# MystenLabs/dapol

Hardware: AMD Instinct MI355X
Metric: entities/sec (tree build + 64-bit range-proof gen), 2^20 leaves, 1/2/4/8 GPU (higher is better)
Workload: dtype int32 limbs (255-bit modular integers)

## Files before the change

dapol_amd/csrc/host_range.inc:

```

#include <cstdlib>
#include "policy_plan.inc"
#include "prove_plan.inc"

struct MsmTiming {
    std::vector<hipEvent_t> ev;
    std::vector<int> kind;
    size_t used = 0;
    bool enabled = false;
    size_t kernels[2] = {0, 0};
    ~MsmTiming() { for (auto e : ev) (void)hipEventDestroy(e); }
    hipError_t mark(hipStream_t st, int k = 0) {
        if (!enabled) return hipSuccess;
        if (used == ev.size()) {
            hipEvent_t e;
            hipError_t r = hipEventCreate(&e);
            if (r != hipSuccess) return r;
            ev.push_back(e);
        }
        if ((used & 1) == 0) { if (kind.size() <= used / 2) kind.push_back(k); else kind[used / 2] = k; }
        return hipEventRecord(ev[used++], st);
    }
    void count(int k, size_t n) { if (enabled) kernels[k] += n; }
    double total_ms(int k) {
// ... 38 lines not shown
static void launch_msm(hipStream_t st, const RangeArgs& A, const TableView& tv, int round, int lpl) {
    const unsigned B = (unsigned)A.B, S = (unsigned)(A.nsplit > 1 ? A.nsplit : 1);
    if (lpl == 8) hipLaunchKernelGGL((k_rp_msm<MSM_PLAIN, 8>), dim3((B + 3) / 4 * S), dim3(64), 0, st, A, tv, round);
    else if (lpl == 4) hipLaunchKernelGGL((k_rp_msm<MSM_PLAIN, 4>), dim3((B + 7) / 8 * S), dim3(64), 0, st, A, tv, round);
    else if (lpl == 2) hipLaunchKernelGGL((k_rp_msm<MSM_PLAIN, 2>), dim3((B + 15) / 16 * S), dim3(64), 0, st, A, tv, round);
    else if (lpl == 16) hipLaunchKernelGGL((k_rp_msm<MSM_PLAIN, 16>), dim3((B + 1) / 2 * S), dim3(64), 0, st, A, tv, round);
    else hipLaunchKernelGGL((k_rp_msm<MSM_PLAIN, 32>), dim3(B * S), dim3(64), 0, st, A, tv, round);
}
static void launch_msm_tail(hipStream_t st, const RangeArgs& At, const TableView& tvt, int round, int lpl) {
    const unsigned B = (unsigned)At.B;
    if (lpl == 2) hipLaunchKernelGGL((k_rp_msm<MSM_TAIL, 2>), dim3((B + 15) / 16), dim3(64), 0, st, At, tvt, round);
    else if (lpl == 1) hipLaunchKernelGGL((k_rp_msm<MSM_TAIL, 1>), dim3((B + 31) / 32), dim3(64), 0, st, At, tvt, round);
    else if (lpl == 32) hipLaunchKernelGGL((k_rp_msm<MSM_TAIL, 32>), dim3(B), dim3(64), 0, st, At, tvt, round);
    else if (lpl == 8) hipLaunchKernelGGL((k_rp_msm<MSM_TAIL, 8>), dim3((B + 3) / 4), dim3(64), 0, st, At, tvt, round);
    else hipLaunchKernelGGL((k_rp_msm<MSM_TAIL, 4>), dim3((B + 7) / 8), dim3(64), 0, st, At, tvt, round);
}

static size_t scratch_budget_bytes(const dapol_ctx* ctx = nullptr) {
    const double GiB = 1024.0 * 1024.0 * 1024.0;
    if (const char* e = knob("DAPOL_SCRATCH_GB")) {
        double gb = atof(e);
        if (gb < 0.25) gb = 0.25;
        return (size_t)(gb * GiB);
    }
    if (ctx && ctx->opt.scratch_gb > 0) return (size_t)((ctx->opt.scratch_gb < 0.25 ? 0.25 : ctx->opt.scratch_gb) * GiB);
    double want = (ctx && ctx->opt.profile == DAPOL_PROFILE_HOST ? 56.0 : 130.0) * GiB;
    size_t free_b = 0, total_b = 0;
    if (hipMemGetInfo(&free_b, &total_b) == hipSuccess) {
        double avail = (double)free_b + (ctx ? (double)ctx->scratch.bytes : 0.0) - 8.0 * GiB;
        if (avail < 0.25 * GiB) avail = 0.25 * GiB;
        if (avail < want) want = avail;
    }
    return (size_t)want;
}


static unsigned fold_blocks(const RangeArgs& A, size_t cb, int round) {
    if (!A.stab) return nblk(cb * (size_t)A.N, 256);
    const size_t half = (size_t)1 << (A.lgN - 1 - round), nt = (round + 1 <= STAB_ROUNDS) ? ((size_t)2 << (round + 1)) : 0;
    return nblk(cb * (half > nt ? half : nt), 256);
}

struct PendingProve {
    dapol_ctx* ctx = nullptr;
    DevBuf<uint32_t> err;
    int pinned_slot = 0;
    uint32_t* h_err_p = nullptr;
    bool armed = false;
    int32_t finish() {
        if (!armed) return DAPOL_OK;
        armed = false;
        HIPCHK(hipStreamSynchronize(ctx->stream));
        if (*h_err_p) return fail(DAPOL_ERR_INVALID_ARGUMENT, "prover drew a zero challenge (ProofError::MaliciousDealer)");
        return DAPOL_OK;
    }
    ~PendingProve() { if (armed) (void)hipStreamSynchronize(ctx->stream); }
};

struct ProveLane {
    RangeArgs A;
    int32_t* split[3];
    int32_t* gsacc;
};
static ProveLane carve_lane(const ProvePlan& P, RangeArgs A, uint8_t* base) {
    ProveLane L{};
    const size_t chunk = P.chunk, N = (size_t)P.N, T = (size_t)P.tail_n;
    size_t o = 0;
    A.a = (sc*)(base + o); o += chunk * N * sizeof(sc);
    A.b = (sc*)(base + o); o += chunk * N * sizeof(sc);
    A.s1 = (sc*)(base + o); o += chunk * N * sizeof(sc);
    A.s2 = (sc*)(base + o); o += chunk * N * sizeof(sc);
    A.dig = (dig_t*)(base + o); o += align_up(chunk * P.dig_elems * sizeof(dig_t), 256);
    A.st = (ProofState*)(base + o); o += align_up(chunk * sizeof(ProofState), 256);
    A.PA = (int32_t*)(base + o); o += chunk * 160;
    A.P0 = (int32_t*)(base + o); o += chunk * 160;
    A.P1 = (int32_t*)(base + o); o += chunk * 160;
    A.tailT = (int32_t*)(base + o); o += chunk * 2 * T * TAIL_ROW_WORDS * 4;
    A.tail_a = (sc*)(base + o); o += chunk * T * sizeof(sc);
    A.tail_b = (sc*)(base + o); o += chunk * T * sizeof(sc);
    A.tail_s1 = (sc*)(base + o); o += chunk * T * sizeof(sc);
    A.tail_s2 = (sc*)(base + o); o += chunk * T * sizeof(sc);
    A.fs_part = (sc*)(base + o); o += chunk * FS_PARTS_MAX * 3 * sizeof(sc);
    A.stab = P.stab_bytes ? (sc*)(base + o) : nullptr; o += chunk * P.stab_bytes;
    L.gsacc = (int32_t*)(base + o); o += chunk * P.acc_bytes;
    o = align_up(o, 256);
    L.split[0] = (int32_t*)(base + o); o += chunk * (size_t)P.part_split() * 160;
    L.split[1] = (int32_t*)(base + o); o += chunk * (size_t)P.part_split() * 160;
    o = align_up(o, 256);
    L.split[2] = (int32_t*)(base + o);
    L.A = A;
    return L;
}

static void launch_main_msm(dapol_ctx* ctx, const ProvePlan& P, const ProveLane& L, const RangeArgs& A, hipStream_t st, int round, MsmTiming* tm) {
    const size_t cb = A.B;
    if (P.gs) {
        const int LW = P.gs_LW;
        const unsigned g_acc = nblk(cb * (size_t)LW, 64);
        const int ns = P.slices_for(cb), slice_rows = A.N / ns, tile = P.tile_for(cb, ns);
        const size_t side_words = (size_t)4 * FE_NL * cb * LW * ns;
        for (int side = 0; side < 2; side++)
            for (int q0 = 0; q0 < slice_rows; q0 += tile) {
                const int nq = slice_rows - q0 < tile ? slice_rows - q0 : tile;
                if (LW < A.nwin)
                    hipLaunchKernelGGL(k_rp_msm_gs_hi, dim3(g_acc, ns), dim3(64), 0, st, A, ctx->tv, round, side, q0, nq, q0 == 0 ? 1 : 0,
                                       L.gsacc + side * side_words, slice_rows, LW);
                else
                    hipLaunchKernelGGL(k_rp_msm_gs, dim3(g_acc, ns), dim3(64), 0, st, A, ctx->tv, round, side, q0, nq, q0 == 0 ? 1 : 0,
                                       L.gsacc + side * side_words, slice_rows);
            }
        if (ns > 1) hipLaunchKernelGGL(k_rp_gs_sum_slices, dim3(nblk(2 * cb * (size_t)LW, 64)), dim3(64), 0, st, A, L.gsacc, side_words, ns, LW);
        hipLaunchKernelGGL(k_rp_gs_combine, dim3(nblk(2 * cb, 64)), dim3(64), 0, st, A, L.gsacc, side_words, ns, LW);
        if (tm) tm->count(0, 2 * (size_t)((slice_rows + tile - 1) / tile));
    } else if (P.part_split() > 1) {
        RangeArgs As = A;
        As.nsplit = P.part_split(); As.P0 = L.split[0]; As.P1 = L.split[1];
        if (P.quad_split) hipLaunchKernelGGL(k_rp_msm_quad, dim3((unsigned)(cb * (size_t)P.quad_split)), dim3(64), 0, st, As, ctx->tv, round);
        else launch_msm(st, As, ctx->tv, round, P.lpl);
        hipLaunchKernelGGL(k_rp_sum_splits, dim3((unsigned)(2 * cb)), dim3(64), 0, st, cb, As.nsplit, As.P0, As.P1, A.P0, A.P1);
    } else {
        launch_msm(st, A, ctx->tv, round, P.lpl);
        if (tm) tm->count(0, 1);
    }
}

static int32_t launch_materialise(dapol_ctx* ctx, const ProvePlan& P, const ProveLane& L, const RangeArgs& A, hipStream_t st, MsmTiming* tm) {
    const size_t cb = A.B, T = (size_t)P.tail_n;
    const unsigned g_tail = (unsigned)(cb * (size_t)(P.tail_n / 32));
    if (P.gs_mat) {
        const int LW = P.mat_LW(), cpl = P.mat_cpl(cb);
        const unsigned g_cls = nblk(cb * (size_t)LW, 64);
        const size_t slot_words = (size_t)4 * FE_NL * cb * LW;
        for (int side = 0; side < 2; side++)
            for (int c0 = 0; c0 < P.tail_n; c0 += MAT_GROUP) {
                const int nc = P.tail_n - c0 < MAT_GROUP ? P.tail_n - c0 : MAT_GROUP;
                for (int c = 0; c < nc; c += cpl) {
                    const int ny = nc - c < cpl ? nc - c : cpl;
                    hipLaunchKernelGGL(k_rp_mat_gs, dim3(g_cls, ny), dim3(64), 0, st, A, ctx->tv, side, c0 + c, 0, LW, L.gsacc + c * slot_words);
                    if (LW < A.nwin) hipLaunchKernelGGL(k_rp_mat_gs, dim3(g_cls, ny), dim3(64), 0, st, A, ctx->tv, side, c0 + c, 1, LW, L.gsacc + c * slot_words);
                }
                hipLaunchKernelGGL(k_rp_mat_gs_horner, dim3(nblk(cb * (size_t)nc, 64)), dim3(64), 0, st, A, side, c0, nc, LW, L.gsacc);
            }
        if (tm) tm->count(1, 2 * (size_t)((P.tail_n + cpl - 1) / cpl) * (LW < A.nwin ? 2 : 1));
    } else if (P.mat_split > 1) {
        RangeArgs Am = A;
        Am.nsplit = P.mat_split; Am.P0 = L.split[2];
        hipLaunchKernelGGL((k_rp_msm<MSM_MATERIALIZE, 32>), dim3(g_tail * (unsigned)P.mat_split), dim3(64), 0, st, Am, ctx->tv, -1); LAUNCH_CHECK();
        hipLaunchKernelGGL(k_rp_sum_mat, dim3(nblk(cb * 2 * T, 64)), dim3(64), 0, st, cb * 2 * T, P.mat_split, Am.P0, A.tailT);
    } else {
        hipLaunchKernelGGL((k_rp_msm<MSM_MATERIALIZE, 32>), dim3(g_tail), dim3(64), 0, st, A, ctx->tv, -1);
        if (tm) tm->count(1, 1);
    }
    LAUNCH_CHECK();
    return DAPOL_OK;
}

static int32_t queue_chunk(dapol_ctx* ctx, const ProvePlan& P, const ProveLane& L, RangeArgs A, hipStream_t st, ForkGuard& fg, uint32_t* d_err,
                           MsmTiming* tm) {
    const size_t cb = A.B;
    const int fs_shape = P.fs_shape, nf_rounds = P.nf_rounds();
    sc* const stab_buf = A.stab;
    if (!P.stab_main) A.stab = nullptr;
    const unsigned g_wave = (unsigned)cb, g_lane = nblk(cb, 64), g_dig = (unsigned)(cb * (size_t)(A.TP / 64));
    const unsigned g_gsdig = nblk(cb * (size_t)(2 * A.N), 64);
    hipLaunchKernelGGL(k_rp_nonce_key, dim3(g_lane), dim3(64), 0, st, A); LAUNCH_CHECK();
    if (P.gs) hipLaunchKernelGGL(k_rp_nonces_gs, dim3(g_gsdig), dim3(64), 0, st, A);
    else hipLaunchKernelGGL(k_rp_nonces, dim3(g_dig), dim3(64), 0, st, A);
    LAUNCH_CHECK();
    if (P.side_A) {
        HIPCHK(hipEventRecord(ctx->ev_fork, st));
        HIPCHK(hipStreamWaitEvent(ctx->side[2], ctx->ev_fork, 0));
        fg.forked(2);
        hipLaunchKernelGGL(k_rp_A, dim3(g_wave), dim3(64), 0, ctx->side[2], A, ctx->tv); LAUNCH_CHECK();
        HIPCHK(hipEventRecord(ctx->ev_join[2], ctx->side[2]));
        FAULT_AFTER_FORK("prove_A");
    } else if (P.a_lane(cb)) {
        hipLaunchKernelGGL(k_rp_A_lane, dim3(g_lane), dim3(64), 0, st, A, ctx->tv); LAUNCH_CHECK();
    } else {
        hipLaunchKernelGGL(k_rp_A, dim3(g_wave), dim3(64), 0, st, A, ctx->tv); LAUNCH_CHECK();
    }
    if (tm) HIPCHK(tm->mark(st));
    launch_main_msm(ctx, P, L, A, st, -1, tm); LAUNCH_CHECK();
    if (tm) HIPCHK(tm->mark(st));
    if (P.side_A) { HIPCHK(hipStreamWaitEvent(st, ctx->ev_join[2], 0)); fg.joined(2); }
    LAUNCH_FS(k_rp_finish1, fs_shape, cb, st, A, ctx->tv); LAUNCH_CHECK();
    hipLaunchKernelGGL(k_rp_poly, dim3(g_wave * (unsigned)A.fs_parts), dim3(64), 0, st, A); LAUNCH_CHECK();
    LAUNCH_FS(k_rp_finish2, fs_shape, cb, st, A, ctx->tv); LAUNCH_CHECK();
    hipLaunchKernelGGL(k_rp_lr, dim3(g_wave * (unsigned)A.fs_parts), dim3(64), 0, st, A); LAUNCH_CHECK();
    if (fs_shape == 2) hipLaunchKernelGGL(k_rp_finish3<2>, dim3(g_wave), dim3(64), 0, st, A);
    else hipLaunchKernelGGL(k_rp_finish3<0>, dim3(g_lane), dim3(64), 0, st, A);
    LAUNCH_CHECK();
    for (int k = 0; k < nf_rounds; k++) {
        if (P.gs) hipLaunchKernelGGL(k_rp_round_prep_gs, dim3(g_gsdig), dim3(64), 0, st, A, k);
        else hipLaunchKernelGGL(k_rp_round_prep, dim3(g_dig), dim3(64), 0, st, A, k);
        LAUNCH_CHECK();
        hipLaunchKernelGGL(k_rp_round_ip, dim3(g_wave), dim3(64), 0, st, A, k); LAUNCH_CHECK();
        if (tm) HIPCHK(tm->mark(st));
        launch_main_msm(ctx, P, L, A, st, k, tm); LAUNCH_CHECK();
        if (tm) HIPCHK(tm->mark(st));
        LAUNCH_FS(k_rp_round_finish, fs_shape, cb, st, A, ctx->tv, k); LAUNCH_CHECK();
        hipLaunchKernelGGL(k_rp_fold, dim3(fold_blocks(A, cb, k)), dim3(256), 0, st, A, k);
        LAUNCH_CHECK();
    }
    if (nf_rounds == A.lgN) {
        hipLaunchKernelGGL(k_rp_final, dim3(g_lane), dim3(64), 0, st, A, d_err); LAUNCH_CHECK();
        return DAPOL_OK;
    }
    if (P.gs_mat) hipLaunchKernelGGL(k_rp_mat_prep_gs, dim3(g_gsdig), dim3(64), 0, st, A);
    else hipLaunchKernelGGL(k_rp_mat_prep, dim3(g_dig), dim3(64), 0, st, A);
    LAUNCH_CHECK();
    if (tm) HIPCHK(tm->mark(st, 1));
    { int32_t rc = launch_materialise(ctx, P, L, A, st, tm); if (rc) return rc; }
    if (tm) HIPCHK(tm->mark(st, 1));
    const unsigned g_tail = (unsigned)(cb * (size_t)(P.tail_n / 32));
    {
        RangeArgs Ai = A;
        Ai.stab = P.stab_tail ? stab_buf : nullptr;
        hipLaunchKernelGGL(k_rp_tail_table, dim3(g_tail), dim3(64), 0, st, Ai); LAUNCH_CHECK();
    }
    RangeArgs At = A;
    At.N = P.tail_n; At.lgN = P.tail_lgn; At.TP = 2 * P.tail_n; At.wbits = TAIL_WBITS; At.nwin = TAIL_NWIN; At.nsplit = 0;
    At.a = A.tail_a; At.b = A.tail_b; At.s1 = A.tail_s1; At.s2 = A.tail_s2;
    At.stab = P.stab_tail ? stab_buf : nullptr;
    At.out_round0 = nf_rounds;
    const TableView tvt{A.tailT, 1, TAIL_WBITS, 0, 0};
    for (int k = 0; k < P.tail_lgn; k++) {
        hipLaunchKernelGGL(k_rp_round_prep, dim3(g_tail), dim3(64), 0, st, At, k); LAUNCH_CHECK();
        hipLaunchKernelGGL(k_rp_round_ip, dim3(g_wave), dim3(64), 0, st, At, k); LAUNCH_CHECK();
        launch_msm_tail(st, At, tvt, k, P.tail_lpl); LAUNCH_CHECK();
        LAUNCH_FS(k_rp_round_finish, fs_shape, cb, st, At, ctx->tv, k); LAUNCH_CHECK();
        hipLaunchKernelGGL(k_rp_fold, dim3(fold_blocks(At, cb, k)), dim3(256), 0, st, At, k);
        LAUNCH_CHECK();
    }
    hipLaunchKernelGGL(k_rp_final, dim3(g_lane), dim3(64), 0, st, At, d_err); LAUNCH_CHECK();
    return DAPOL_OK;
}

static int32_t range_prove_device(dapol_ctx* ctx, int n, int m, size_t B, const uint64_t* d_vals, const uint32_t* d_blind,
                                  const uint32_t* d_Vc, const uint32_t* d_seed, const uint64_t* d_stream, uint64_t slot_base,
                                  const uint32_t* d_tape, uint32_t* d_out, MsmTiming* tm, size_t tape_stride = 0, uint32_t sub_k = 1,
                                  size_t out_stride = 0, PendingProve* pend = nullptr) {
    ProveShape s{};
    s.n = n; s.m = m; s.B = B;
    s.tail_length = ctx->opt.tail_length; s.small_call_max = ctx->opt.small_call_max; s.generator_stationary = ctx->opt.generator_stationary;
    s.streams = ctx->opt.streams; s.gs_tile_rows = ctx->opt.gs_tile_rows; s.gs_slices = ctx->opt.gs_slices; s.chunk_proofs = ctx->opt.chunk_proofs;
    s.wbits = ctx->tv.wbits; s.nwin = ctx->tv.nwin_c(); s.hi_split = ctx->tv.hi_split;
    s.n_cu = ctx->n_cu; s.resident_waves = ctx->resident_waves();
    s.budget_bytes = scratch_budget_bytes(ctx);
    s.timed = tm != nullptr;
    ProvePlan P = plan_range_prove(s);
    for (bool lowered = false;; lowered = true) {
        hipError_t e = ctx->scratch.ensure(P.lane_bytes() * P.nlanes);
        if (e == hipSuccess) {
            if (lowered) P.finalise(s, P.chunk, P.nlanes);
            break;
        }
        (void)hipGetLastError();
        if (e != hipErrorOutOfMemory || (P.nlanes == 1 && P.chunk <= 64)) return fail_hip(e, "scratch allocation", __FILE__, __LINE__);
        if (P.nlanes > 1) P.nlanes--;
        else P.chunk = (P.chunk + 1) / 2;
    }
    const size_t chunk = P.chunk, slots = (size_t)m * (2 * (size_t)n + 4);
    const int nlanes = P.nlanes;
    RangeArgs A{};
    A.n = n; A.m = m; A.N = P.N; A.lgN = P.lgN; A.TP = P.TP;
    A.out_words = 72 + 16 * A.lgN;
    A.seed = d_seed; A.slot_base = slot_base;
    A.wbits = s.wbits; A.nwin = s.nwin;
    A.tail_n = P.tail_n; A.use_hi = P.use_hi ? 1 : 0; A.fs_parts = P.fs_parts; A.mat_round = P.nf_rounds();
    A.stream_id = d_stream;
    A.tape_stride = (uint32_t)(tape_stride ? tape_stride : slots);
    A.tape = d_tape;
    A.sub_k = sub_k ? sub_k : 1; A.sub_slots = (uint32_t)slots;
    A.out = d_out; A.out_stride = out_stride ? out_stride : (size_t)A.out_words;
    ProveLane lanes[4];
    hipStream_t lane_stream[4] = {ctx->stream, ctx->side[0], ctx->side[1], ctx->side[2]};
    for (int ln = 0; ln < nlanes; ln++) lanes[ln] = carve_lane(P, A, (uint8_t*)ctx->scratch.p + P.lane_bytes() * ln);
    DevBuf<uint32_t> err_own;
    DevBuf<uint32_t>& err = pend ? pend->err : err_own;
    HIPCHK(err.alloc(1));
    HIPCHK(hipMemsetAsync(err.p, 0, 4, ctx->stream));
    ForkGuard fg(ctx);
    if (nlanes > 1) {
        HIPCHK(hipEventRecord(ctx->ev_fork, ctx->stream));
        for (int ln = 1; ln < nlanes; ln++) { HIPCHK(hipStreamWaitEvent(lane_stream[ln], ctx->ev_fork, 0)); fg.forked(ln - 1); }
    }
    size_t chunk_no = 0;
    for (size_t first = 0; first < B; first += chunk, chunk_no++) {
        const int ln = (int)(chunk_no % (size_t)nlanes);
        if (chunk_no == 2) FAULT_AFTER_FORK("prove_lanes");
        RangeArgs Ac = lanes[ln].A;
        Ac.B = B - first < chunk ? B - first : chunk;
        Ac.vals = d_vals + first * m;
        Ac.blind = d_blind + first * m * 8;
        Ac.Vc = d_Vc + first * m * 8;
        Ac.p0 = first;
        int32_t rc = queue_chunk(ctx, P, lanes[ln], Ac, lane_stream[ln], fg, err.p, tm);
        if (rc) return rc;
    }
    for (int ln = 1; ln < nlanes; ln++) {
        HIPCHK(hipEventRecord(ctx->ev_join[ln - 1], lane_stream[ln]));
        HIPCHK(hipStreamWaitEvent(ctx->stream, ctx->ev_join[ln - 1], 0));
        fg.joined(ln - 1);
    }
    if (pend) {
        pend->ctx = ctx;
        pend->h_err_p = ctx->h_pinned + pend->pinned_slot;
        HIPCHK(hipMemcpyAsync(pend->h_err_p, err.p, 4, hipMemcpyDeviceToHost, ctx->stream));
        pend->armed = true;
        return DAPOL_OK;
    }
    uint32_t h_err = 0;
// ... 52 lines not shown
```

dapol_amd/csrc/kernels_range.h:

```cpp
#pragma once
#include <hip/hip_runtime.h>
#include <type_traits>
#include "kernels_ctx_tree.h"
#include "ge_quad.h"

namespace dapol {

struct ProofState {
    uint64_t strobe[25];
    uint32_t pos, pos_begin;
    uint32_t err, pad_;
    sc y, z, y_inv, x, w, u, u_inv;
    sc a_bl, s_bl, t1, t2, t1_bl, t2_bl, t_x, cL, cR;
    uint32_t nkey[8];
};

struct RangeArgs {
    int n, m, N, lgN, TP;
    int wbits, nwin;
    size_t B;
    const uint64_t* vals;
    const uint32_t* blind;
    const uint32_t* Vc;
    const uint32_t* seed;
// ... 380 lines not shown
            fe qel;
            for (int i = 0; i < FE_NL; i++) qel.v[i] = e[i];
            quad_madd(c, ql, qel, neg);
        }
    }
    for (int off = 16; off >= 4; off >>= 1) {
        fe o;
        for (int i = 0; i < FE_NL; i++) o.v[i] = __shfl_down(c.v[i], off, 64);
        quad_add(c, ql, o);
    }
    if (sub == 0) {
        int32_t* dst = (side ? A.P1 : A.P0) + (b * nsplit + split) * 40 + FE_NL * ql;
        for (int i = 0; i < FE_NL; i++) dst[i] = c.v[i];
    }
}

__global__ __launch_bounds__(64) void k_rp_sum_splits(size_t B, int nsplit, const int32_t* PS0, const int32_t* PS1, int32_t* P0, int32_t* P1) {
    const size_t t = blockIdx.x;
    if (t >= 2 * B) return;
    const size_t b = t >> 1;
    const int l = threadIdx.x;
    const int32_t* src = ((t & 1) ? PS1 : PS0) + b * (size_t)nsplit * 40;
    ge_p3 acc;
    if (l < nsplit) ld_p3(acc, src + (size_t)l * 40);
    else ge_identity(acc);
    for (int s = l + 64; s < nsplit; s += 64) {
        ge_p3 p, r;
        ld_p3(p, src + (size_t)s * 40);
        ge_add(r, acc, p);
        acc = r;
    }
    wave_reduce_point(acc, nsplit < 64 ? nsplit : 64);
    if (l == 0) st_p3(((t & 1) ? P1 : P0) + b * 40, acc);
}

__global__ __launch_bounds__(64) void k_rp_sum_mat(size_t n_gen, int nsplit, const int32_t* PS, int32_t* tailT) {
    size_t g = (size_t)blockIdx.x * 64 + threadIdx.x;
    if (g >= n_gen) return;
    const int32_t* src = PS + g * (size_t)nsplit * 40;
    ge_p3 acc, p, r;
    ld_p3(acc, src);
    for (int s = 1; s < nsplit; s++) {
        ld_p3(p, src + (size_t)s * 40);
        ge_add(r, acc, p);
        acc = r;
    }
    st_p3(tailT + g * TAIL_ROW_WORDS, acc);
}

template <int ENTRIES>
__device__ __forceinline__ void build_niels_row(int32_t* row) {
    ge_p3 base, mul;
    ld_p3(base, row);
    mul = base;
    fe pre[ENTRIES - 1];
#pragma unroll
    for (int e = 1; e < ENTRIES; e++) {
        if (e > 1) { ge_p3 t; ge_add(t, mul, base); mul = t; }
        int32_t* slot = row + e * 32;
        for (int i = 0; i < FE_NL; i++) { slot[i] = mul.X.v[i]; slot[FE_NL + i] = mul.Y.v[i]; slot[2 * FE_NL + i] = mul.Z.v[i]; }
        if (e == 1) pre[0] = mul.Z;
        else fe_mul(pre[e - 1], pre[e - 2], mul.Z);
    }
    fe inv;
    fe_invert(inv, pre[ENTRIES - 2]);
#pragma unroll
    for (int e = ENTRIES - 1; e >= 1; e--) {
        int32_t* slot = row + e * 32;
        fe X, Y, Z, zi, x, y;
        for (int i = 0; i < FE_NL; i++) { X.v[i] = slot[i]; Y.v[i] = slot[FE_NL + i]; Z.v[i] = slot[2 * FE_NL + i]; }
        if (e > 1) { fe_mul(zi, inv, pre[e - 2]); fe t; fe_mul(t, inv, Z); inv = t; }
        else zi = inv;
        fe_mul(x, X, zi);
        fe_mul(y, Y, zi);
        ge_niels q;
        ge_to_niels(q, x, y);
        niels_store_entry(slot, q);
    }
    ge_niels id;
    ge_niels_identity(id);
    niels_store_entry(row, id);
}

__global__ __launch_bounds__(64) void k_rp_tail_table(RangeArgs A) {
    const int T = A.tail_n, bpp = (2 * T) >> 6;
    size_t b = blockIdx.x / bpp;
    int g = (int)(blockIdx.x % bpp) * 64 + threadIdx.x;
    build_niels_row<TAIL_ENTRIES>(A.tailT + (b * (size_t)(2 * T) + g) * TAIL_ROW_WORDS);
    sc one, v;
    sc_zero(one); one.v[0] = 1;
    int i = g < T ? g : g - T;
    if (g == 0) stab_init(A, b);
    st_sc((g < T ? A.tail_s1 : A.tail_s2) + b * T + i, one);
    ld_sc(v, (g < T ? A.a : A.b) + b * A.N + i);
    st_sc((g < T ? A.tail_a : A.tail_b) + b * T + i, v);
}

__global__ __launch_bounds__(64) void k_rp_mat_prep(RangeArgs A) {
    int nch = A.TP >> 6;
    size_t b = blockIdx.x / nch;
    int ch = blockIdx.x % nch, l = threadIdx.x, side = l >> 5, q = 32 * ch + (l & 31), pos = 64 * ch + l;
    if (q >= A.N) { zero_digits(A, b, pos); return; }
    sc s;
    coeff_plain(s, A, b, A.mat_round, q, side != 0);
    write_digits_plain(A, b, pos, s.v);
}

__device__ __forceinline__ void st_load(Strobe& s, const ProofState& p) {
    for (int i = 0; i < 25; i++) s.s[i] = p.strobe[i];
    s.pos = p.pos;
    s.pos_begin = p.pos_begin;
}
__device__ __forceinline__ void st_store(ProofState& p, const Strobe& s) {
    for (int i = 0; i < 25; i++) p.strobe[i] = s.s[i];
    p.pos = s.pos;
    p.pos_begin = s.pos_begin;
}
__device__ __forceinline__ void st_load(WStrobe& s, const ProofState& p) {
    s.a = s.l < 25 ? p.strobe[s.l < 25 ? s.l : 0] : 0;
    s.pos = p.pos;
    s.pos_begin = p.pos_begin;
}
__device__ __forceinline__ void st_store(ProofState& p, const WStrobe& s) {
    if (s.l < 25) p.strobe[s.l] = s.a;
    if (s.l == 0) { p.pos = s.pos; p.pos_begin = s.pos_begin; }
}
template <class S>
__device__ __forceinline__ void challenge_scalar(sc& r, S& s, const char* label, int n) {
    uint32_t w[16];
    merlin_challenge_wide(s, label, n, w);
    sc_from_wide(r, w);
}
template <class S>
__device__ __forceinline__ void append_scalar(S& s, const char* label, int n, const uint32_t* canon8) {
    merlin_append_words(s, label, n, canon8, 8);
}
__device__ __forceinline__ void fs_scalar(sc& r, const RangeArgs& A, size_t b, int which) {
    const ProofState& ps = A.st[b];
    if (A.fs_parts > 1) {
        sc_zero(r);
        for (int w = 0; w < A.fs_parts; w++) {
            sc t;
            ld_sc(t, A.fs_part + (b * A.fs_parts + w) * 3 + which);
            sc_add(r, r, t);
        }
    } else {
        r = which == 0 ? ps.t1 : which == 1 ? ps.t2 : ps.t_x;
    }
}
template <int MODE> struct FsShape {
    using strobe_t = typename std::conditional<MODE == 2, WStrobe, Strobe>::type;
    const int l;
    size_t b;
    bool valid;
    int h_lo, h_hi;
    __device__ FsShape(const RangeArgs& A) : l((int)threadIdx.x) {
        const size_t t_ = (size_t)blockIdx.x * 64 + threadIdx.x;
        b = MODE == 2 ? (size_t)blockIdx.x : (MODE == 1 ? t_ >> 1 : t_);
        valid = b < A.B;
        if (!valid) b = A.B - 1;
        if (MODE == 0) { h_lo = 0; h_hi = 2; }
        else if (MODE == 1) { h_lo = (int)(t_ & 1); h_hi = h_lo + 1; }
        else { h_lo = l >> 5; h_hi = h_lo + 1; }
    }
    __device__ void share(uint32_t* first8, uint32_t* second8) const {
        if (MODE == 1) { for (int i = 0; i < 8; i++) second8[i] = (uint32_t)__shfl_down((int)second8[i], 1, 64); }
        if (MODE == 2) {
            for (int i = 0; i < 8; i++) { first8[i] = (uint32_t)__shfl((int)first8[i], 0, 64); second8[i] = (uint32_t)__shfl((int)second8[i], 32, 64); }
        }
    }
    __device__ bool point_lane() const { return MODE == 2 ? (l & 31) == 0 : true; }
    __device__ bool owns_transcript() const { return MODE == 2 ? true : (MODE == 1 ? ((l & 1) == 0 && valid) : valid); }
    __device__ bool writes() const { return MODE == 2 ? l == 0 : true; }
    __device__ void begin(strobe_t& s) const { if constexpr (MODE == 2) wstrobe_lanes(s, l); }
};
template <int MODE>
__device__ __forceinline__ void blinding_sum(sc& bl, const RangeArgs& A, size_t b, uint32_t slot0, uint32_t stride, int lane) {
    sc t;
// ... 472 lines not shown
```

dapol_amd/csrc/kernels_range_gs.h:

```cpp
#pragma once
#include "kernels_range.h"

namespace dapol {

__device__ __forceinline__ void write_digits_gs(const RangeArgs& A, size_t p, int sp, const uint32_t* c) {
    const size_t L = A.B * (size_t)A.nwin;
    int32_t* out = reinterpret_cast<int32_t*>(A.dig) + ((((size_t)(sp >> 2)) * L + p) << 2) + (sp & 3);
    const size_t wstride = A.B * (size_t)4;
    const int W = A.wbits, NW = A.nwin, half = 1 << (W - 1);
    const uint32_t mask = (1u << W) - 1;
    uint32_t x[8];
#pragma unroll
    for (int i = 0; i < 8; i++) x[i] = c[i];
    int carry = 0;
#pragma nounroll
    for (int w = 0; w < NW; w++) {
        const int b = (int)(x[0] & mask) + carry;
        carry = (b >= half && w != NW - 1) ? 1 : 0;
        out[(size_t)w * wstride] = b - (carry << W);
#pragma unroll
        for (int i = 0; i < 7; i++) x[i] = (x[i] >> W) | (x[i + 1] << (32 - W));
        x[7] >>= W;
    }
}
// ... 183 lines not shown
enum { GS_ACC_SLOTS = 32, GS_MAX_SLICES = 16, GS_FULL_LANES = 3072 * 64 };
static_assert(GS_ACC_SLOTS >= MAT_GROUP && GS_ACC_SLOTS >= 2 * GS_MAX_SLICES, "accumulator slots");

__global__ __launch_bounds__(64) void k_rp_mat_prep_gs(RangeArgs A) {
    GS_BLOCKS(A, vb) {
        size_t p;
        int sp;
        if (!gs_thread(A, vb, p, sp)) continue;
        const int side = sp >= A.N ? 1 : 0, rem = sp - side * A.N;
        const int per = A.N / A.tail_n, cls = rem / per, k = rem - cls * per;
        sc s;
        coeff_plain(s, A, p, A.mat_round, cls + k * A.tail_n, side != 0);
        write_digits_gs(A, p, sp, s.v);
    }
}

__global__ __launch_bounds__(64, DAPOL_GS_OCC) void k_rp_mat_gs(RangeArgs A, TableView tbl, int side, int cls, int hi, int LW, int32_t* __restrict__ accs) {
    const size_t LM = A.B * (size_t)LW, L = A.B * (size_t)A.nwin;
    const size_t lane = (size_t)blockIdx.x * 64 + threadIdx.x;
    if (lane >= LM) return;
    cls += (int)blockIdx.y;
    accs += (size_t)blockIdx.y * 4 * FE_NL * LM;
    const int w = (int)(lane / A.B);
    const size_t p = lane - (size_t)w * A.B;
    const int wd = w + (hi ? LW : 0);
    if (wd >= A.nwin) return;
    ge_p3 acc;
    int32_t* ap = accs + lane;
    if (!hi) ge_identity(acc);
    else {
#pragma unroll
        for (int i = 0; i < FE_NL; i++) {
            acc.X.v[i] = ap[(size_t)i * LM]; acc.Y.v[i] = ap[(size_t)(FE_NL + i) * LM];
            acc.Z.v[i] = ap[(size_t)(2 * FE_NL + i) * LM]; acc.T.v[i] = ap[(size_t)(3 * FE_NL + i) * LM];
        }
    }
    const int per = A.N / A.tail_n;
    const dapol_v4i* dg = reinterpret_cast<const dapol_v4i*>(A.dig) + ((size_t)(side * A.N + cls * per) >> 2) * L + (size_t)wd * A.B + p;
    dapol_v4i d4 = dg[0], dn = d4;
#pragma nounroll
    for (int k = 0; k < per; k++) {
        if ((k & 3) == 0 && k + 4 < per) dn = dg[(size_t)((k >> 2) + 1) * L];
        const int d = d4.x;
        d4.x = d4.y; d4.y = d4.z; d4.z = d4.w;
        if ((k & 3) == 3) d4 = dn;
        const int row = gen_row(tbl, A.n, cls + k * A.tail_n, side != 0);
        tbl_madd(acc, tbl, hi ? tbl.row_hi(row) : row, d);
    }
#pragma unroll
    for (int i = 0; i < FE_NL; i++) {
        ap[(size_t)i * LM] = acc.X.v[i]; ap[(size_t)(FE_NL + i) * LM] = acc.Y.v[i];
        ap[(size_t)(2 * FE_NL + i) * LM] = acc.Z.v[i]; ap[(size_t)(3 * FE_NL + i) * LM] = acc.T.v[i];
    }
}

__global__ __launch_bounds__(64) void k_rp_mat_gs_horner(RangeArgs A, int side, int cls0, int ncls, int LW, const int32_t* __restrict__ accs) {
    const size_t LM = A.B * (size_t)LW;
    const size_t t = (size_t)blockIdx.x * 64 + threadIdx.x;
    if (t >= (size_t)ncls * A.B) return;
    const int c = (int)(t / A.B);
    const size_t p = t - (size_t)c * A.B;
    const int32_t* slot = accs + (size_t)c * 4 * FE_NL * LM;
    auto load = [&](ge_p3& r, int w) {
        const int32_t* ap = slot + (size_t)w * A.B + p;
        for (int i = 0; i < FE_NL; i++) {
            r.X.v[i] = ap[(size_t)i * LM]; r.Y.v[i] = ap[(size_t)(FE_NL + i) * LM];
            r.Z.v[i] = ap[(size_t)(2 * FE_NL + i) * LM]; r.T.v[i] = ap[(size_t)(3 * FE_NL + i) * LM];
        }
    };
    ge_p3 acc, q, r;
    load(acc, LW - 1);
#pragma nounroll
    for (int w = LW - 2; w >= 0; w--) {
#pragma nounroll
        for (int d = 0; d < A.wbits; d++) ge_dbl(acc, acc, d == A.wbits - 1);
        load(q, w);
        ge_add(r, acc, q);
        acc = r;
    }
    const int T = A.tail_n;
    st_p3(A.tailT + (p * (size_t)(2 * T) + (size_t)(side * T + cls0 + c)) * TAIL_ROW_WORDS, acc);
}

}
```

dapol_amd/csrc/prove_plan.inc:

```
#pragma once
#include <cstddef>
#include <cstdint>
#include <cstdlib>

enum { FS_PARTS_MAX = 8 };

struct ProveShape {
    int n, m;
    size_t B;
    int tail_length, small_call_max, generator_stationary, streams, gs_tile_rows, gs_slices;
    long long chunk_proofs;
    int wbits, nwin, hi_split;
    int n_cu;
    size_t resident_waves;
    size_t budget_bytes;
    bool timed;
};

struct ProvePlan {
    int N, lgN, TP;
    int nwin, hi_split;
    int tail_n, tail_lgn;
    bool small_call, use_hi;
    int fs_shape, fs_parts;
    bool gs, gs_mat;
    int gs_LW, acc_slots;
    bool stab_main, stab_tail;
    int msm_split, mat_split, quad_split;
    size_t dig_elems, stab_bytes, acc_bytes, per_proof, split_bytes;
    size_t chunk;
    int nlanes;
    bool big_batch;
    int lpl, tail_lpl;
    bool side_A;
    int gs_tile, gs_slices_forced, mat_cpl_forced;
    bool gs_tile_set, a_lane_ok;
    const char* lpl_env;

    int part_split() const { return quad_split ? quad_split : msm_split; }
    int nf_rounds() const { return lgN - tail_lgn; }
    size_t lane_bytes() const { return (chunk * per_proof + 8192 + split_bytes + 4095) / 4096 * 4096; }

    int slices_for(size_t cb) const {
        if (gs_slices_forced) return gs_slices_forced <= acc_slots / 2 ? gs_slices_forced : acc_slots / 2;
        int ns = cb <= 4096 ? 16 : (cb < 40000 ? 8 : (cb < 65536 ? 4 : 1));
        if (N < 1024) {
            const size_t lanes = cb * (size_t)gs_LW;
            ns = lanes >= 2 * (size_t)GS_FULL_LANES ? 1 : (lanes >= (size_t)GS_FULL_LANES ? 2 : (lanes >= (size_t)GS_FULL_LANES / 2 ? 4 : (lanes >= (size_t)GS_FULL_LANES / 8 ? 8 : 16)));
        }
        while (ns > 1 && ((N / ns) % 4 != 0 || N / ns < 32)) ns /= 2;
        return ns;
    }
    int tile_for(size_t cb, int ns) const {
        int tile = (!gs_tile_set && cb * (size_t)nwin < 2 * (size_t)GS_FULL_LANES && N / ns >= 32) ? 32 : gs_tile;
        if (gs_LW < nwin && !gs_tile_set) tile = tile / 2;
        return tile;
    }
    int mat_LW() const { return hi_split ? hi_split : nwin; }
    int mat_cpl(size_t cb) const {
        if (mat_cpl_forced) return mat_cpl_forced;
        int cpl = 1;
        while (cpl < MAT_GROUP && cb * (size_t)mat_LW() * (size_t)cpl < GS_FULL_LANES) cpl *= 2;
        return cpl;
    }
    bool a_lane(size_t cb) const { return !side_A && gs && N < 1024 && cb >= 4096 && a_lane_ok; }

    void finalise(const ProveShape& s, size_t chunk_, int nlanes_);
};

static int small_split_cap(bool use_hi) {
    if (const char* e = knob("DAPOL_SMALL_SPLIT")) { int v = atoi(e); if (v >= 1 && v <= 64 && !(v & (v - 1))) return v; }
    return use_hi ? 64 : 8;
}
static size_t quad_max_waves(size_t dflt) {
    if (const char* e = knob("DAPOL_QUAD_MAX_WAVES")) { long long v = atoll(e); if (v > 0) return (size_t)v; }
    return dflt;
}
static int pick_lanes_per_list(size_t proofs, int terms_per_list, int nwin, int wbits, const int* cand, int ncand, size_t resident, size_t n_simd,
                               bool shared_simd = false) {
    int best = cand[0];
    double best_cost = 1e300;
    const size_t occ = n_simd ? (resident + n_simd - 1) / n_simd : 1;
    for (int i = 0; i < ncand; i++) {
        int lpl = cand[i];
        size_t waves = (proofs + (size_t)(32 / lpl) - 1) / (size_t)(32 / lpl);
        const size_t full = waves / resident, rem = waves % resident;
        const size_t krem = rem ? (rem + n_simd - 1) / (n_simd ? n_simd : 1) : 0;
        double per_simd = (double)(full * occ) + (double)krem;
        if (shared_simd) per_simd = (double)full * (1.0 + 0.23 * (double)(occ - 1)) + (krem ? 1.0 + 0.23 * (double)(krem - 1) : 0.0);
        double per_lane = (double)((terms_per_list + lpl - 1) / lpl) * nwin * (shared_simd && lpl == 32 ? 2.0 : 1.0) + (double)nwin * wbits;
        double cost = per_simd * per_lane;
        if (cost < best_cost) { best_cost = cost; best = lpl; }
    }
    return best;
}
static int tail_lanes_per_list(bool small_call, const char* e ) {
    if (e) { int v = atoi(e); if (v == 1 || v == 2 || v == 4 || v == 8 || v == 32) return v; }
    if (small_call) return 32;
    return 2;
}
static int msm_lanes_per_list(int N, bool big_batch = false, const char* e = knob("DAPOL_LPL")) {
    if (e) { int v = atoi(e); if (v == 2 || v == 4 || v == 8 || v == 16 || v == 32) return v; }
    return N >= 1024 ? (big_batch ? 2 : 8) : (N >= 256 ? 16 : 32);
}

static ProvePlan plan_range_prove(const ProveShape& s) {
    ProvePlan P{};
    const size_t B = s.B;
    const int N = s.n * s.m;
    P.N = N;
    while ((1 << P.lgN) < N) P.lgN++;
    P.TP = 2 * N < 64 ? 64 : 2 * N;
    P.nwin = s.nwin; P.hi_split = s.hi_split;
    const int lgN = P.lgN;
    int tail_n = 64;
    if (s.tail_length > 0) tail_n = s.tail_length;
    const char* const e_tail_n = knob("DAPOL_TAIL_N");
    if (e_tail_n) { int v = atoi(e_tail_n); if (v == 32 || v == 64 || v == 128 || v == 256) tail_n = v; }
    if (lgN < 8 || s.tail_length < 0 || knob("DAPOL_NO_TAIL")) tail_n = 0;
    const char* const e_gs = knob("DAPOL_GS");
    const int gs_env = e_gs ? (atoi(e_gs) != 0 ? 1 : 0) : -1;
    size_t gs_small_min = N == 64 ? 2048 : (N == 128 ? 1024 : 512);
    if (const char* e = knob("DAPOL_GS_SMALL_MIN")) { long long v = atoll(e); if (v >= 64) gs_small_min = (size_t)v; }
    const bool gs_small = N >= 64 && N < 1024 && N % 4 == 0 && B >= gs_small_min && s.generator_stationary == 0 && gs_env < 0;
    if (gs_small && N < 512 && !e_tail_n) tail_n = 0;
    if (gs_small && N == 512 && tail_n == 64 && s.tail_length == 0 && !e_tail_n) tail_n = 32;
    size_t small_max = s.small_call_max > 0 ? (size_t)s.small_call_max : 8191;
    const char* const e_small_max = knob("DAPOL_SMALL_MAX");
    if (e_small_max) { long long v = atoll(e_small_max); if (v >= 1) small_max = (size_t)v; }
    size_t gs_min = 1024;
    if (const char* e = knob("DAPOL_GS_MIN")) { long long v = atoll(e); if (v >= 1) gs_min = (size_t)v; }
    const bool gs_shape = N >= 1024 && N % 4 == 0 && s.generator_stationary >= 0 && gs_env != 0;
    if (gs_shape && s.small_call_max <= 0 && !e_small_max && small_max >= gs_min) small_max = gs_min - 1;
    const char* const e_lpl = knob("DAPOL_LPL");
    P.lpl_env = e_lpl;
    const bool small_call = B <= small_max && N >= 256 && !e_lpl && !knob("DAPOL_NO_SPLIT") && !gs_small;
    const bool use_hi = small_call && s.hi_split && !knob("DAPOL_NO_SMALL_HI");
    P.small_call = small_call; P.use_hi = use_hi;
    P.fs_shape = !small_call ? (B <= 1536 ? 2 : (B <= 16384 ? 1 : 0)) : (B <= 256 ? 2 : 1);
    if (knob("DAPOL_NO_PAIR")) P.fs_shape = 0;
    if (const char* e = knob("DAPOL_FS_SHAPE")) { int v = atoi(e); if (v >= 0 && v <= 2) P.fs_shape = v; }
    if (use_hi && B <= 32 && !knob("DAPOL_SMALL_TAIL")) tail_n = 0;
    while (tail_n && 4 * tail_n > N) tail_n >>= 1;
    if (tail_n && tail_n < 32) tail_n = 0;
    int tail_lgn = 0;
    while (tail_n && (1 << tail_lgn) < tail_n) tail_lgn++;
    P.tail_n = tail_n; P.tail_lgn = tail_lgn;
    const size_t T = (size_t)tail_n;
    size_t dig_elems = (size_t)s.nwin * P.TP;
    if (dig_elems < (size_t)TAIL_NWIN * 2 * T) dig_elems = (size_t)TAIL_NWIN * 2 * T;
    P.dig_elems = dig_elems;
    const bool no_stab = knob("DAPOL_NO_STAB") != nullptr;
    P.stab_main = !no_stab && (tail_n ? lgN - tail_lgn : lgN - 1) <= STAB_ROUNDS;
    P.stab_tail = !no_stab && tail_n && tail_lgn - 1 <= STAB_ROUNDS;
    bool gs_possible = (!small_call && N % 4 == 0 && N >= 1024 && B >= gs_min) || gs_small;
    if (s.generator_stationary) gs_possible = s.generator_stationary > 0 && !small_call && N % 4 == 0 && N >= 64;
    if (gs_env >= 0) gs_possible = gs_env != 0 && !small_call && N % 4 == 0 && N >= 64;
    int acc_slots = GS_ACC_SLOTS;
    if (N < 1024) {
        acc_slots = 2 * (N / 32 < GS_MAX_SLICES ? N / 32 : GS_MAX_SLICES);
        if (tail_n && acc_slots < MAT_GROUP) acc_slots = MAT_GROUP;
    }
    P.acc_slots = acc_slots;
    P.acc_bytes = gs_possible ? (size_t)acc_slots * s.nwin * 4 * FE_NL * 4 : 0;
    P.stab_bytes = (P.stab_main || P.stab_tail) ? (size_t)2 * 2 * STAB_N * sizeof(sc) : 0;
    P.per_proof = 4 * (size_t)N * sizeof(sc) + dig_elems * sizeof(dig_t) + (sizeof(ProofState) + 15) / 16 * 16 + 3 * 160 +
                  2 * T * TAIL_ROW_WORDS * 4 + 4 * T * sizeof(sc) + FS_PARTS_MAX * 3 * sizeof(sc) + P.stab_bytes + P.acc_bytes;
    int nlanes = s.streams > 0 ? s.streams : 1;
    if (const char* e = knob("DAPOL_STREAMS")) { int v = atoi(e); if (v >= 1 && v <= 4) nlanes = v; }
    size_t chunk = s.budget_bytes / nlanes / P.per_proof;
    if (chunk < 1) chunk = 1;
    if (chunk > B) chunk = B;
    {
        const char* const e_chunk = knob("DAPOL_CHUNK");
        const bool chunk_set = e_chunk || s.chunk_proofs > 0;
        const long long chunk_forced = e_chunk ? atoll(e_chunk) : s.chunk_proofs;
        const size_t rw = s.resident_waves;
        size_t ppw = 16;
        if (e_lpl) { int v = atoi(e_lpl); if (v == 2 || v == 4 || v == 8) ppw = (size_t)(32 / v); }
        const size_t big_chunk = (3 * rw * ppw <= chunk) ? 3 * rw * ppw : ((2 * rw * ppw <= chunk) ? 2 * rw * ppw : rw * ppw), std_chunk = 5 * rw * 4;
        P.big_batch = !chunk_set && N >= 1024 && B >= big_chunk && chunk >= big_chunk;
        size_t cap = chunk_set ? (size_t)chunk_forced : (P.big_batch ? big_chunk : std_chunk);
        const size_t small_unit = rw * 64 / (size_t)(s.hi_split ? s.hi_split : s.nwin);
        if (gs_small && !chunk_set) cap = 8 * small_unit;
        if (cap < 64) cap = 64;
        if (chunk > cap) chunk = cap;
        if (gs_small && !chunk_set && chunk > small_unit) chunk -= chunk % small_unit;
    }
    while (nlanes > 1 && chunk * (size_t)(nlanes - 1) >= B) nlanes--;
    P.chunk = chunk; P.nlanes = nlanes;
    bool gs = P.big_batch || (!small_call && B >= gs_min && chunk >= 1024 && N >= 1024 && N % 4 == 0) || (gs_small && chunk >= 64);
    if (s.generator_stationary) gs = s.generator_stationary > 0 && !small_call && N % 4 == 0 && N >= 64;
    if (gs_env >= 0) gs = gs_env != 0 && !small_call && N % 4 == 0 && N >= 64;
    if (!gs_possible) gs = false;
    P.gs = gs;
    P.gs_mat = gs && tail_n && (N / tail_n) % 4 == 0 && !knob("DAPOL_NO_GS_MAT");
    P.gs_tile = s.gs_tile_rows > 0 ? s.gs_tile_rows : 16;
    const char* const e_tile = knob("DAPOL_GS_TILE");
    P.gs_tile_set = s.gs_tile_rows > 0 || e_tile;
    if (e_tile) { int v = atoi(e_tile); if (v >= 4 && v % 4 == 0) P.gs_tile = v; }
    P.gs_slices_forced = (s.gs_slices > 0 && N % (4 * s.gs_slices) == 0 && N / s.gs_slices >= 4) ? s.gs_slices : 0;
    if (const char* e = knob("DAPOL_GS_SLICES")) { int v = atoi(e); if ((v == 1 || v == 2 || v == 4 || v == 8 || v == 16) && N % (4 * v) == 0 && N / v >= 4) P.gs_slices_forced = v; }
    P.gs_LW = (gs && N < 1024 && s.hi_split && !knob("DAPOL_NO_GS_HI")) ? s.hi_split : s.nwin;
    if (const char* e = knob("DAPOL_GS_MAT_CPL")) { int v = atoi(e); if (v >= 1 && v <= MAT_GROUP) P.mat_cpl_forced = v; }
    P.a_lane_ok = !knob("DAPOL_NO_A_LANE");
    P.msm_split = 1; P.mat_split = 1;
    if (small_call) {
        const int cap = small_split_cap(use_hi), min_terms = use_hi ? 1 : 4;
        while (P.msm_split < cap && (size_t)P.msm_split * 2 * B <= 2048 && N / 32 / (P.msm_split * 2) >= min_terms) P.msm_split *= 2;
        if (tail_n && !knob("DAPOL_NO_SPLIT_MAT"))
            while (P.mat_split < 8 && (size_t)(P.mat_split * 2) * B * (size_t)(tail_n / 32) <= 4096 && N / tail_n / (P.mat_split * 2) >= 2) P.mat_split *= 2;
    }
    P.fs_parts = 1;
    if (small_call && B <= 64 && !knob("DAPOL_NO_FS_PARTS")) {
        const int iters = (N + 63) / 64;
        while (P.fs_parts < FS_PARTS_MAX && iters / (P.fs_parts * 2) >= 2) P.fs_parts *= 2;
    }
    if (use_hi && P.msm_split > 1 && (size_t)P.msm_split * 4 * B <= quad_max_waves(2048) && N % (8 * P.msm_split * 4) == 0 && !knob("DAPOL_NO_QUAD")) P.quad_split = P.msm_split * 4;
    P.split_bytes = (P.part_split() > 1 ? (2 * chunk * (size_t)P.part_split() * 160 + 255) / 256 * 256 : 0) +
                    (P.mat_split > 1 ? (chunk * 2 * T * (size_t)P.mat_split * 160 + 255) / 256 * 256 : 0);
    P.finalise(s, chunk, nlanes);
    return P;
}

void ProvePlan::finalise(const ProveShape& s, size_t chunk_, int nlanes_) {
    chunk = chunk_; nlanes = nlanes_;
    const char* const e_tail_lpl = knob("DAPOL_TAIL_LPL");
    lpl = msm_lanes_per_list(N, big_batch, lpl_env);
    tail_lpl = tail_lanes_per_list(small_call, e_tail_lpl);
    if (small_call) lpl = 32;
    else if (!lpl_env && N >= 1024 && !big_batch && chunk < 32768) {
        const int cand[2] = {8, 16};
        lpl = pick_lanes_per_list(chunk, N, s.nwin, s.wbits, cand, 2, s.resident_waves, (size_t)s.n_cu * 4);
    }
    if (!e_tail_lpl && !small_call && tail_n && chunk < 65536) {
        const int cand[4] = {2, 4, 8, 32};
        tail_lpl = pick_lanes_per_list(chunk, tail_n, TAIL_NWIN, TAIL_WBITS, cand, 4, s.resident_waves, (size_t)s.n_cu * 4, true);
    }
    side_A = small_call && nlanes == 1 && s.B <= 64 && !s.timed && !knob("DAPOL_NO_SIDE_A");
}
```

Measured before the change: 58030.

## Add generator-stationary tail MSM and batched-inversion tail table build

Adds two alternative paths for the tail rounds of the range proof. The first is a per-window accumulator kernel (k_rp_tail_gs), where each thread walks all terms for one window, followed by a combine kernel that does the doubling and add chain across windows. The second is a tail table builder that handles four rows per lane and shares one field inversion across them via Montgomery's trick. Both are enabled only for large GS batches (chunk ≥ 65536) and aim to cut inversion count and MSM overhead in the tail. The cost is extra record buffer space in some configurations and more register pressure per thread.

```diff
diff --git a/dapol_amd/csrc/host_range.inc b/dapol_amd/csrc/host_range.inc
--- a/dapol_amd/csrc/host_range.inc
+++ b/dapol_amd/csrc/host_range.inc
@@ -144,7 +144,7 @@
     A.tail_s2 = (sc*)(base + o); o += chunk * T * sizeof(sc);
     A.fs_part = (sc*)(base + o); o += chunk * FS_PARTS_MAX * 3 * sizeof(sc);
     A.stab = P.stab_bytes ? (sc*)(base + o) : nullptr; o += chunk * P.stab_bytes;
-    L.gsacc = (int32_t*)(base + o); o += chunk * P.acc_bytes;
+    L.gsacc = (int32_t*)(base + o); o += chunk * (P.acc_bytes + P.tail_rec_bytes);
     o = align_up(o, 256);
     L.split[0] = (int32_t*)(base + o); o += chunk * (size_t)P.part_split() * 160;
     L.split[1] = (int32_t*)(base + o); o += chunk * (size_t)P.part_split() * 160;
@@ -278,7 +278,9 @@
     {
         RangeArgs Ai = A;
         Ai.stab = P.stab_tail ? stab_buf : nullptr;
-        hipLaunchKernelGGL(k_rp_tail_table, dim3(g_tail), dim3(64), 0, st, Ai); LAUNCH_CHECK();
+        if (P.tail_rpl == 4) hipLaunchKernelGGL(k_rp_tail_table4, dim3(nblk(cb * (size_t)(2 * P.tail_n / 4), 64)), dim3(64), 0, st, Ai);
+        else hipLaunchKernelGGL(k_rp_tail_table, dim3(g_tail), dim3(64), 0, st, Ai);
+        LAUNCH_CHECK();
     }
     RangeArgs At = A;
     At.N = P.tail_n; At.lgN = P.tail_lgn; At.TP = 2 * P.tail_n; At.wbits = TAIL_WBITS; At.nwin = TAIL_NWIN; At.nsplit = 0;
@@ -289,7 +291,11 @@
     for (int k = 0; k < P.tail_lgn; k++) {
         hipLaunchKernelGGL(k_rp_round_prep, dim3(g_tail), dim3(64), 0, st, At, k); LAUNCH_CHECK();
         hipLaunchKernelGGL(k_rp_round_ip, dim3(g_wave), dim3(64), 0, st, At, k); LAUNCH_CHECK();
-        launch_msm_tail(st, At, tvt, k, P.tail_lpl); LAUNCH_CHECK();
+        if (P.tail_gs) {
+            hipLaunchKernelGGL(k_rp_tail_gs, dim3(nblk(2 * cb, TAIL_GS_LISTS)), dim3(TAIL_GS_BLOCK), 0, st, At, tvt, k, L.gsacc); LAUNCH_CHECK();
+            hipLaunchKernelGGL(k_rp_tail_combine, dim3(nblk(2 * cb, 64)), dim3(64), 0, st, At, L.gsacc);
+        } else launch_msm_tail(st, At, tvt, k, P.tail_lpl);
+        LAUNCH_CHECK();
         LAUNCH_FS(k_rp_round_finish, fs_shape, cb, st, At, ctx->tv, k); LAUNCH_CHECK();
         hipLaunchKernelGGL(k_rp_fold, dim3(fold_blocks(At, cb, k)), dim3(256), 0, st, At, k);
         LAUNCH_CHECK();
diff --git a/dapol_amd/csrc/kernels_range.h b/dapol_amd/csrc/kernels_range.h
--- a/dapol_amd/csrc/kernels_range.h
+++ b/dapol_amd/csrc/kernels_range.h
@@ -486,11 +486,8 @@
     niels_store_entry(row, id);
 }
 
-__global__ __launch_bounds__(64) void k_rp_tail_table(RangeArgs A) {
-    const int T = A.tail_n, bpp = (2 * T) >> 6;
-    size_t b = blockIdx.x / bpp;
-    int g = (int)(blockIdx.x % bpp) * 64 + threadIdx.x;
-    build_niels_row<TAIL_ENTRIES>(A.tailT + (b * (size_t)(2 * T) + g) * TAIL_ROW_WORDS);
+__device__ __forceinline__ void tail_row_vectors(const RangeArgs& A, size_t b, int g) {
+    const int T = A.tail_n;
     sc one, v;
     sc_zero(one); one.v[0] = 1;
     int i = g < T ? g : g - T;
@@ -498,6 +495,85 @@
     st_sc((g < T ? A.tail_s1 : A.tail_s2) + b * T + i, one);
     ld_sc(v, (g < T ? A.a : A.b) + b * A.N + i);
     st_sc((g < T ? A.tail_a : A.tail_b) + b * T + i, v);
+}
+__global__ __launch_bounds__(64) void k_rp_tail_table(RangeArgs A) {
+    const int T = A.tail_n, bpp = (2 * T) >> 6;
+    size_t b = blockIdx.x / bpp;
+    int g = (int)(blockIdx.x % bpp) * 64 + threadIdx.x;
+    build_niels_row<TAIL_ENTRIES>(A.tailT + (b * (size_t)(2 * T) + g) * TAIL_ROW_WORDS);
+    tail_row_vectors(A, b, g);
+}
+
+template <int ENTRIES>
+__device__ __forceinline__ void niels_row_multiples(int32_t* row, fe& total) {
+    ge_p3 base, mul;
+    ld_p3(base, row);
+    mul = base;
+#pragma nounroll
+    for (int e = 1; e < ENTRIES; e++) {
+        if (e > 1) { ge_p3 t; ge_add(t, mul, base); mul = t; }
+        int32_t* slot = row + e * 32;
+        for (int i = 0; i < FE_NL; i++) { slot[i] = mul.X.v[i]; slot[FE_NL + i] = mul.Y.v[i]; slot[2 * FE_NL + i] = mul.Z.v[i]; }
+        if (e == 1) total = mul.Z;
+        else { fe t; fe_mul(t, total, mul.Z); total = t; }
+    }
+}
+template <int ENTRIES>
+__device__ __forceinline__ void niels_row_finish(int32_t* row, fe inv) {
+    fe pre[ENTRIES - 1];
+#pragma unroll
+    for (int e = 1; e < ENTRIES; e++) {
+        const int32_t* slot = row + e * 32;
+        fe Z;
+        for (int i = 0; i < FE_NL; i++) Z.v[i] = slot[2 * FE_NL + i];
+        if (e == 1) pre[0] = Z;
+        else fe_mul(pre[e - 1], pre[e - 2], Z);
+    }
+#pragma unroll
+    for (int e = ENTRIES - 1; e >= 1; e--) {
+        int32_t* slot = row + e * 32;
+        fe X, Y, Z, zi, x, y;
+        for (int i = 0; i < FE_NL; i++) { X.v[i] = slot[i]; Y.v[i] = slot[FE_NL + i]; Z.v[i] = slot[2 * FE_NL + i]; }
+        if (e > 1) { fe_mul(zi, inv, pre[e - 2]); fe t; fe_mul(t, inv, Z); inv = t; }
+        else zi = inv;
+        fe_mul(x, X, zi);
+        fe_mul(y, Y, zi);
+        ge_niels q;
+        ge_to_niels(q, x, y);
+        niels_store_entry(slot, q);
+    }
+    ge_niels id;
+    ge_niels_identity(id);
+    niels_store_entry(row, id);
+}
+__global__ __launch_bounds__(64) void k_rp_tail_table4(RangeArgs A) {
+    const int T = A.tail_n, LP = (2 * T) >> 2;
+    const size_t t = (size_t)blockIdx.x * 64 + threadIdx.x;
+    const size_t b = t / (size_t)LP;
+    if (b >= A.B) return;
+    const int g0 = (int)(t - b * (size_t)LP);
+    int32_t* rows = A.tailT + b * (size_t)(2 * T) * TAIL_ROW_WORDS;
+    fe t0, t1, t2, t3;
+#pragma nounroll
+    for (int k = 0; k < 4; k++) {
+        fe tot;
+        niels_row_multiples<TAIL_ENTRIES>(rows + (size_t)(g0 + k * LP) * TAIL_ROW_WORDS, tot);
+        if (k == 0) t0 = tot; else if (k == 1) t1 = tot; else if (k == 2) t2 = tot; else t3 = tot;
+    }
+    fe p01, p23, all, inv, i01, i23;
+    fe_mul(p01, t0, t1);
+    fe_mul(p23, t2, t3);
+    fe_mul(all, p01, p23);
+    fe_invert(inv, all);
+    fe_mul(i01, inv, p23);
+    fe_mul(i23, inv, p01);
+#pragma nounroll
+    for (int k = 0; k < 4; k++) {
+        fe ri;
+        fe_mul(ri, k < 2 ? i01 : i23, k == 0 ? t1 : (k == 1 ? t0 : (k == 2 ? t3 : t2)));
+        niels_row_finish<TAIL_ENTRIES>(rows + (size_t)(g0 + k * LP) * TAIL_ROW_WORDS, ri);
+        tail_row_vectors(A, b, g0 + k * LP);
+    }
 }
 
 __global__ __launch_bounds__(64) void k_rp_mat_prep(RangeArgs A) {
diff --git a/dapol_amd/csrc/kernels_range_gs.h b/dapol_amd/csrc/kernels_range_gs.h
--- a/dapol_amd/csrc/kernels_range_gs.h
+++ b/dapol_amd/csrc/kernels_range_gs.h
@@ -289,4 +289,47 @@
     st_p3(A.tailT + (p * (size_t)(2 * T) + (size_t)(side * T + cls0 + c)) * TAIL_ROW_WORDS, acc);
 }
 
-}
+enum { TAIL_GS_BLOCK = 256, TAIL_GS_LISTS = TAIL_GS_BLOCK / TAIL_NWIN, TAIL_REC_WORDS = 4 * FE_NL };
+static_assert(TAIL_GS_LISTS >= 1, "a list's windows fit a block");
+__global__ __launch_bounds__(TAIL_GS_BLOCK, DAPOL_GS_OCC) void k_rp_tail_gs(RangeArgs A, TableView tbl, int round, int32_t* __restrict__ recs) {
+    const int li = (int)threadIdx.x / TAIL_NWIN, w = (int)threadIdx.x - li * TAIL_NWIN;
+    const size_t list = (size_t)blockIdx.x * TAIL_GS_LISTS + li;
+    if (li >= TAIL_GS_LISTS || list >= 2 * A.B) return;
+    const size_t p = list >> 1;
+    const int side = (int)(list & 1);
+    tbl.base += p * (size_t)(2 * A.N) * tbl.row_words();
+    const dig_t* dw = A.dig + (p * A.nwin + (size_t)w) * (size_t)A.TP + 32 * side;
+    ge_p3 acc;
+    ge_identity(acc);
+    dapol_v4i d4 = *reinterpret_cast<const dapol_v4i*>(dw), dn = d4;
+#pragma nounroll
+    for (int q = 0; q < A.N; q++) {
+        if ((q & 3) == 0 && q + 4 < A.N) dn = *reinterpret_cast<const dapol_v4i*>(dw + 64 * ((q + 4) >> 5) + ((q + 4) & 31));
+        const int d = d4.x;
+        d4.x = d4.y; d4.y = d4.z; d4.z = d4.w;
+        if ((q & 3) == 3) d4 = dn;
+        bool isH;
+        const int j = term_generator(round, A.N, A.lgN, side, q, isH);
+        tbl_madd(acc, tbl, j + (isH ? A.N : 0), d);
+    }
+    st_p3(recs + (list * TAIL_NWIN + (size_t)w) * TAIL_REC_WORDS, acc);
+}
+
+__global__ __launch_bounds__(64) void k_rp_tail_combine(RangeArgs A, const int32_t* __restrict__ recs) {
+    const size_t list = (size_t)blockIdx.x * 64 + threadIdx.x;
+    if (list >= 2 * A.B) return;
+    const int32_t* rp = recs + list * TAIL_NWIN * TAIL_REC_WORDS;
+    ge_p3 acc, t2, r;
+    ld_p3(acc, rp + (size_t)(A.nwin - 1) * TAIL_REC_WORDS);
+#pragma nounroll
+    for (int w = A.nwin - 2; w >= 0; w--) {
+#pragma nounroll
+        for (int d = 0; d < A.wbits; d++) ge_dbl(acc, acc, d == A.wbits - 1);
+        ld_p3(t2, rp + (size_t)w * TAIL_REC_WORDS);
+        ge_add(r, acc, t2);
+        acc = r;
+    }
+    st_p3(((list & 1) ? A.P1 : A.P0) + (list >> 1) * 40, acc);
+}
+
+}
diff --git a/dapol_amd/csrc/prove_plan.inc b/dapol_amd/csrc/prove_plan.inc
--- a/dapol_amd/csrc/prove_plan.inc
+++ b/dapol_amd/csrc/prove_plan.inc
@@ -4,6 +4,8 @@
 #include <cstdlib>
 
 enum { FS_PARTS_MAX = 8 };
+enum { TAIL_RPL_DEFAULT = 4 };
+enum { TAIL_GS_DEFAULT = 1 };
 
 struct ProveShape {
     int n, m;
@@ -33,6 +35,10 @@
     bool big_batch;
     int lpl, tail_lpl;
     bool side_A;
+    bool tail_gs;
+    int tail_order;
+    size_t tail_rec_bytes;
+    int tail_rpl, tail_rpl_forced;
     int gs_tile, gs_slices_forced, mat_cpl_forced;
     bool gs_tile_set, a_lane_ok;
     const char* lpl_env;
@@ -103,6 +109,8 @@
     if (e) { int v = atoi(e); if (v == 2 || v == 4 || v == 8 || v == 16 || v == 32) return v; }
     return N >= 1024 ? (big_batch ? 2 : 8) : (N >= 256 ? 16 : 32);
 }
+
+static size_t tail_rec_need() { return (size_t)2 * TAIL_NWIN * 4 * FE_NL * 4; }
 
 static ProvePlan plan_range_prove(const ProveShape& s) {
     ProvePlan P{};
@@ -164,8 +172,11 @@
     P.acc_slots = acc_slots;
     P.acc_bytes = gs_possible ? (size_t)acc_slots * s.nwin * 4 * FE_NL * 4 : 0;
     P.stab_bytes = (P.stab_main || P.stab_tail) ? (size_t)2 * 2 * STAB_N * sizeof(sc) : 0;
+    if (const char* e = knob("DAPOL_TAIL_ORDER")) P.tail_order = (e[0] == 'g' && e[1] == 's' && !e[2]) ? 1 : ((e[0] == 'p' && e[1] == 's' && !e[2]) ? -1 : 0);
+    if (const char* e = knob("DAPOL_TAIL_ROWS_PER_LANE")) { int v = atoi(e); if (v == 1 || v == 4) P.tail_rpl_forced = v; }
+    P.tail_rec_bytes = (P.tail_order > 0 && tail_n && P.acc_bytes < tail_rec_need()) ? tail_rec_need() - P.acc_bytes : 0;
     P.per_proof = 4 * (size_t)N * sizeof(sc) + dig_elems * sizeof(dig_t) + (sizeof(ProofState) + 15) / 16 * 16 + 3 * 160 +
-                  2 * T * TAIL_ROW_WORDS * 4 + 4 * T * sizeof(sc) + FS_PARTS_MAX * 3 * sizeof(sc) + P.stab_bytes + P.acc_bytes;
+                  2 * T * TAIL_ROW_WORDS * 4 + 4 * T * sizeof(sc) + FS_PARTS_MAX * 3 * sizeof(sc) + P.stab_bytes + P.acc_bytes + P.tail_rec_bytes;
     int nlanes = s.streams > 0 ? s.streams : 1;
     if (const char* e = knob("DAPOL_STREAMS")) { int v = atoi(e); if (v >= 1 && v <= 4) nlanes = v; }
     size_t chunk = s.budget_bytes / nlanes / P.per_proof;
@@ -237,5 +248,8 @@
         const int cand[4] = {2, 4, 8, 32};
         tail_lpl = pick_lanes_per_list(chunk, tail_n, TAIL_NWIN, TAIL_WBITS, cand, 4, s.resident_waves, (size_t)s.n_cu * 4, true);
     }
+    tail_gs = tail_n != 0 && (tail_order > 0 || (tail_order == 0 && TAIL_GS_DEFAULT && gs && !small_call && N >= 1024 && chunk >= 65536 && acc_bytes >= tail_rec_need()));
+    tail_rpl = tail_rpl_forced ? tail_rpl_forced : ((TAIL_RPL_DEFAULT == 4 && gs && !small_call && N >= 1024 && chunk >= 65536) ? 4 : 1);
+    if (!tail_n || (2 * tail_n) % 4 != 0) tail_rpl = 1;
     side_A = small_call && nlanes == 1 && s.B <= 64 && !s.timed && !knob("DAPOL_NO_SIDE_A");
 }
```

After: 58930 (median of 6 runs). +1.5%, better.
